# m4rch1n0/vqvae

Measured on AMD Instinct MI355X. Metric: latents/sec through geodesic kNN+APSP+K-medoids, higher is better.
Workload: dtype f64-exact(u32 fixed point)

## Files before the change

vqvae_amd/csrc/geo_common.h:

```cpp
#pragma once
#include <hip/hip_runtime.h>

#include <cstdarg>
#include <cstdint>
#include <cstdio>

#include "geo_hip.h"

namespace geo {

void set_error(const char *fmt, ...);

#define GEO_HIP_CHECK(expr)                                                                      \
    do {                                                                                         \
        hipError_t _e = (expr);                                                                  \
        if (_e != hipSuccess) {                                                                  \
            geo::set_error("%s failed: %s (%s:%d)", #expr, hipGetErrorString(_e), __FILE__, __LINE__); \
            return GEO_E_HIP;                                                                    \
        }                                                                                        \
    } while (0)

#define GEO_REQUIRE(cond, ...)              \
    do {                                    \
        if (!(cond)) {                      \
            geo::set_error(__VA_ARGS__);    \
            return GEO_E_ARG;               \
        }                                   \
    } while (0)

#define GEO_LAUNCH_CHECK() GEO_HIP_CHECK(hipGetLastError())

struct Options {
    int sssp_sb = -1, sssp_act = 1, sssp_sparse_div = -1, sssp_map_div = -1, sssp_group = 1, sssp_grouped_cap = 256,
        sssp_trace = 0, sssp_u32 = 1, sssp_push = 1 ,
        sssp_delta = 8 , sssp_order = 0 , sssp_push_blocks = 64, knn_filter = 1, kpp_grid = 256, kpp_profile = 0, jvp_mid = 0 ,
        jvp_back_valu = 0, jvp_front_valu = 0, jvp_per_node = 1 ,
        jvp_pipe_grid = 1 ,
        jvp_node_jacobian = 1 ,
        jvp_start_dedup = 1 ;
};
Options &options();

static inline size_t align_up(size_t x, size_t a = 256) { return (x + a - 1) / a * a; }

struct Arena {
    char *base;
    size_t size, off;
    Arena(void *p, size_t n) : base(static_cast<char *>(p)), size(n), off(0) {}
    template <typename T>
    T *take(size_t count) {
        size_t bytes = align_up(count * sizeof(T));
        if (off + bytes > size) return nullptr;
        T *r = reinterpret_cast<T *>(base + off);
        off += bytes;
        return r;
    }
};

size_t scan_tmp_bytes(int64_t n);
int exclusive_scan_i32(const int32_t *in, int32_t *out, int64_t n, void *tmp, size_t tmp_bytes,
                       int64_t *total_host, hipStream_t stream);

static inline int grid_for(int64_t work_items, int per_block, int cap = 8192) {
    int64_t g = (work_items + per_block - 1) / per_block;
    if (g < 1) g = 1;
    if (g > cap) g = cap;
    return static_cast<int>(g);
}

}
```

vqvae_amd/csrc/jvp.hip:

```cpp
#include "geo_common.h"

#include <cmath>
#include <cstdlib>
#include <type_traits>
#include <vector>

namespace {

constexpr int TS = 32;
constexpr int NC = 128;
constexpr int MAX_BLOCKS = 4;
constexpr int FRONT_MAX_N1 = 1024;
constexpr int BACK_TS = 8;

typedef float f32x16 __attribute__((ext_vector_type(16)));
typedef __bf16 bf16x8 __attribute__((ext_vector_type(8)));
typedef unsigned short u16x8 __attribute__((ext_vector_type(8)));

struct Shape {
    int d, c0, c1, c2, co, s_out, pad3, p_out;
    int n1, n2;
    int opix_per_chunk, n_chunks;
};

// ... 31 lines not shown
        else b01[n] = (float)(s + (double)b1[co]);
    }
}

__global__ __launch_bounds__(256) void pack_mid_kernel(const float *__restrict__ w2, int c1, int c2, ChunkTable tab,
                                                      int n_chunks, int opix_per_chunk, float *__restrict__ B2p) {
    const size_t per_blk = (size_t)c1 * NC;
    const size_t total = (size_t)n_chunks * MAX_BLOCKS * per_blk;
    for (size_t i = (size_t)blockIdx.x * blockDim.x + threadIdx.x; i < total; i += (size_t)gridDim.x * blockDim.x) {
        const int col = (int)(i % NC);
        const int ci = (int)((i / NC) % c1);
        const int blk = (int)((i / per_blk) % MAX_BLOCKS);
        const int ch = (int)(i / (per_blk * MAX_BLOCKS));
        float v = 0.0f;
        const int lo = col / c2, co = col % c2;
        if (blk < tab.nblk[ch] && lo < opix_per_chunk) {
            const int op = tab.opix[ch][lo], ip = tab.ipix[ch][blk];
            const int ky = (op >> 2) + 1 - 2 * (ip >> 1), kx = (op & 3) + 1 - 2 * (ip & 1);
            if (ky >= 0 && ky < 4 && kx >= 0 && kx < 4) v = w2[(((size_t)ci * c2 + co) * 4 + ky) * 4 + kx];
        }
        B2p[i] = v;
    }
}

__global__ __launch_bounds__(256) void pack_back_kernel(const float *__restrict__ w3, int c2, int co_n,
                                                       float *__restrict__ W3p) {
    const int total = 16 * co_n * c2;
    for (int i = blockIdx.x * blockDim.x + threadIdx.x; i < total; i += gridDim.x * blockDim.x) {
        const int ci = i % c2, co = (i / c2) % co_n, t = i / (c2 * co_n);
        W3p[i] = w3[(((size_t)ci * co_n + co) * 4 + (t >> 2)) * 4 + (t & 3)];
    }
}

template <int DMAX>
__global__ __launch_bounds__(256) void front_kernel(const float *__restrict__ z, const int32_t *__restrict__ src,
                                                   const int32_t *__restrict__ dst, const float *__restrict__ z_start,
                                                   const float *__restrict__ z_end, int64_t e_base, int64_t n_edges,
                                                   int batch, int tiles_per_group, int d, int n1,
                                                   const float *__restrict__ M01, const float *__restrict__ b01,
                                                   float *__restrict__ pre, float *__restrict__ tpre,
                                                   double *__restrict__ partial, int want_stats, int unit_d = 0) {
    __shared__ __attribute__((aligned(8))) float zp[DMAX][TS];
    __shared__ __attribute__((aligned(8))) float dz[DMAX][TS];
    typedef float f32x2 __attribute__((ext_vector_type(2)));
    __shared__ int valid_s[TS];
    __shared__ double ps[FRONT_MAX_N1][4];
    const int tile = blockIdx.x;
    const int group = tile / tiles_per_group, tg = tile % tiles_per_group;
    const int chunk = group >> 1, side = group & 1;
    for (int i = threadIdx.x; i < TS * d; i += 256) {
        const int s = i / d, k = i % d;
        const int within = tg * TS + s;
        const int64_t e = e_base + (int64_t)chunk * batch + within;
        float a = 0.f, b = 0.f;
        const bool ok = within < batch && e < n_edges;
        if (ok) {
            if (src) {
                a = z[(int64_t)src[e] * d + k];
                b = z[(int64_t)dst[e] * d + k];
            } else {
                a = z_start[e * d + k];
                b = z_end[e * d + k];
            }
        }
        zp[k][s] = side == 0 ? a : b;
        dz[k][s] = unit_d ? ((ok && k == (int)(e % unit_d)) ? 1.f : 0.f) : b - a;
        if (k == 0) valid_s[s] = ok ? 1 : 0;
    }
    for (int i = threadIdx.x; i < TS * (DMAX - d); i += 256) {
        const int s = i / (DMAX - d), k = d + i % (DMAX - d);
        zp[k][s] = 0.f;
        dz[k][s] = 0.f;
    }
    __syncthreads();
    const size_t slot0 = (size_t)tile * TS;
    for (int n = threadIdx.x; n < n1; n += 256) {
        float m[DMAX];
#pragma unroll
        for (int k = 0; k < DMAX; ++k) m[k] = k < d ? M01[(size_t)k * n1 + n] : 0.f;
        const float bias = b01[n];
        double sx = 0, sxx = 0, st = 0, sxt = 0;
        for (int s = 0; s < TS; s += 2) {
            f32x2 x2 = {bias, bias}, t2 = {0.f, 0.f};
#pragma unroll
            for (int k = 0; k < DMAX; ++k) {
                const f32x2 mk = {m[k], m[k]};
                x2 = __builtin_elementwise_fma(*reinterpret_cast<const f32x2 *>(&zp[k][s]), mk, x2);
                t2 = __builtin_elementwise_fma(*reinterpret_cast<const f32x2 *>(&dz[k][s]), mk, t2);
            }
#pragma unroll
            for (int u = 0; u < 2; ++u) {
                const float x = u ? x2.y : x2.x, t = u ? t2.y : t2.x;
                pre[(slot0 + s + u) * n1 + n] = x;
                tpre[(slot0 + s + u) * n1 + n] = t;
                if (valid_s[s + u]) {
                    sx += x; sxx += (double)x * x; st += t; sxt += (double)x * t;
                }
            }
        }
        if (want_stats) { ps[n][0] = sx; ps[n][1] = sxx; ps[n][2] = st; ps[n][3] = sxt; }
    }
    if (want_stats) {
        __syncthreads();
        const int c1 = n1 / 4;
        for (int c = threadIdx.x; c < c1; c += 256) {
            double a0 = 0, a1 = 0, a2 = 0, a3 = 0;
#pragma unroll
            for (int px = 0; px < 4; ++px) { a0 += ps[px * c1 + c][0]; a1 += ps[px * c1 + c][1]; a2 += ps[px * c1 + c][2]; a3 += ps[px * c1 + c][3]; }
            double *p = partial + ((size_t)tile * c1 + c) * 4;
            p[0] = a0; p[1] = a1; p[2] = a2; p[3] = a3;
        }
    }
}

template <int DMAX>
__global__ __launch_bounds__(256) void front_mfma_kernel(const float *__restrict__ z, const int32_t *__restrict__ src,
                                                        const int32_t *__restrict__ dst, const float *__restrict__ z_start,
                                                        const float *__restrict__ z_end, int64_t e_base, int64_t n_edges,
                                                        int batch, int tiles_per_group, int d, int n1,
                                                        const float *__restrict__ M01, const float *__restrict__ b01,
                                                        float *__restrict__ pre, float *__restrict__ tpre,
                                                        double *__restrict__ partial, int want_stats) {
    __shared__ float zp[TS][DMAX + 1];
    __shared__ float dz[TS][DMAX + 1];
    __shared__ int valid_s[TS];
    __shared__ double ps[FRONT_MAX_N1][4];
    const int tile = blockIdx.x;
    const int group = tile / tiles_per_group, tg = tile % tiles_per_group;
    const int chunk = group >> 1, side = group & 1;
    for (int i = threadIdx.x; i < TS * DMAX; i += 256) {
        const int s = i / DMAX, k = i % DMAX;
        const int within = tg * TS + s;
        const int64_t e = e_base + (int64_t)chunk * batch + within;
        float a = 0.f, b = 0.f;
        const bool ok = within < batch && e < n_edges;
        if (ok && k < d) {
            if (src) {
                a = z[(int64_t)src[e] * d + k];
                b = z[(int64_t)dst[e] * d + k];
            } else {
                a = z_start[e * d + k];
                b = z_end[e * d + k];
            }
        }
// ... 701 lines not shown
#pragma unroll
            for (int w = 0; w < 4; ++w) { a0 += red[w0 + 2 * w][l][0]; a1 += red[w0 + 2 * w][l][1]; a2 += red[w0 + 2 * w][l][2]; a3 += red[w0 + 2 * w][l][3]; }
            double *p = partial2 + ((size_t)tile * c2 + threadIdx.x) * 4;
            p[0] = a0; p[1] = a1; p[2] = a2; p[3] = a3;
        }
    }
#ifdef GEO_MID_PROF
    { const unsigned long long t_e = __builtin_amdgcn_s_memtime();
      GEO_MP_ADD(6, t_e - mp_prev); GEO_MP_ADD(5, mp_wait); GEO_MP_ADD(7, 1); }
#endif
}

struct Bn2Sums { double sx = 0, sxx = 0, st = 0, sxt = 0; };
__device__ __forceinline__ void bn2_add(Bn2Sums &a, float x, float t, bool live) {
    const double xd = live ? (double)x : 0.0, td = live ? (double)t : 0.0;
    a.sx += xd; a.sxx = fma(xd, xd, a.sxx); a.st += td; a.sxt = fma(xd, td, a.sxt);
}
__device__ __forceinline__ void bn2_store(Bn2Sums a, double *__restrict__ partial2, int tile, int wslot, int co, int lane) {
    a.sx += __shfl_xor(a.sx, 32, 64); a.sxx += __shfl_xor(a.sxx, 32, 64);
    a.st += __shfl_xor(a.st, 32, 64); a.sxt += __shfl_xor(a.sxt, 32, 64);
    if (lane < 32) {
        double *pp = partial2 + (((size_t)tile * 4 + wslot) * 64 + co) * 4;
        pp[0] = a.sx; pp[1] = a.sxx; pp[2] = a.st; pp[3] = a.sxt;
    }
}

template <bool END_ONLY>
__global__ __launch_bounds__(512, 2) void mid_pipe_kernel(const float *__restrict__ pre1, const float *__restrict__ tpre1,
                                                         const NormConst *__restrict__ consts1, int consts_per_group,
                                                         int tiles_per_group, int n_tiles, int ,
                                                         const unsigned short *__restrict__ B3, const float *__restrict__ b2,
                                                         float *__restrict__ pre2, float *__restrict__ tpre2,
                                                         double *__restrict__ partial2, int want_stats, int64_t e_base,
                                                         int64_t n_edges, int batch) {
    constexpr int C1 = 128, LDK = C1 + 8, KS = C1 / 16, NL = 4, c2 = 64;
    typedef float f32x2 __attribute__((ext_vector_type(2)));
    __shared__ __attribute__((aligned(16))) unsigned short A3[2][3][2][TS][LDK];
    const int lane = threadIdx.x & 63, wave = __builtin_amdgcn_readfirstlane((int)(threadIdx.x >> 6));
    const int wq = wave & 3, wg = wave >> 2;
    constexpr int n1 = 4 * C1, n2 = 16 * c2;
    const int r = lane & 31, h = lane >> 5;
    const int k0p = 2 * lane;
    const int lo = wq >> 1, co = (wq & 1) * 32 + r;
    const float bias = b2[co];
    const unsigned v_out = (unsigned)(4 * h * n2 + co) * 4u;
    const int my_tiles = (n_tiles - (int)blockIdx.x + (int)gridDim.x - 1) / (int)gridDim.x;
    if (my_tiles <= 0) return;

    f32x16 accp[NL], acct[NL];
    auto zero_acc = [&]() {
#pragma unroll
        for (int lc = 0; lc < NL; ++lc)
#pragma unroll
            for (int i = 0; i < 16; ++i) { accp[lc][i] = 0.f; acct[lc][i] = 0.f; }
    };
    zero_acc();
    NormConst kA, kB;
    f32x2 rp[4], rt[4];
    auto phys = [&](int t) { return END_ONLY ? ((t / tiles_per_group) * 2 + 1) * tiles_per_group + t % tiles_per_group : t; };
    auto load_consts = [&](int tile) {
        tile = phys(tile);
        const NormConst *kp = consts1 + (size_t)(consts_per_group ? tile / tiles_per_group : 0) * C1 + k0p;
        kA = kp[0];
        kB = kp[1];
    };
    const unsigned v_pair = (unsigned)k0p * 4u;
    auto fetch = [&](int tile, int px, int sample0, auto ns_tag) {
        constexpr int NS = decltype(ns_tag)::value;
        const size_t tbase = (size_t)phys(tile) * TS * n1;
        const __amdgpu_buffer_rsrc_t rp_src = __builtin_amdgcn_make_buffer_rsrc(const_cast<float *>(pre1 + tbase), 0, TS * n1 * 4, 0x00020000);
        const __amdgpu_buffer_rsrc_t rt_src = __builtin_amdgcn_make_buffer_rsrc(const_cast<float *>(tpre1 + tbase), 0, TS * n1 * 4, 0x00020000);
        const int soff = (sample0 * n1 + MidGeom::pix(px) * C1) * 4;
#pragma unroll
        for (int i = 0; i < NS; ++i) {
            rp[i] = __builtin_bit_cast(f32x2, __builtin_amdgcn_raw_buffer_load_b64(rp_src, v_pair, soff + i * n1 * 4, 0));
            rt[i] = __builtin_bit_cast(f32x2, __builtin_amdgcn_raw_buffer_load_b64(rt_src, v_pair, soff + i * n1 * 4, 0));
        }
        __builtin_amdgcn_sched_group_barrier(0x020, 2 * NS, 0);
    };
    auto stage = [&](int buf, int sample0, auto ns_tag) {
        constexpr int NS = decltype(ns_tag)::value;
        unsigned w_idx = (unsigned)((buf * 3 * 2 * TS + sample0) * LDK + k0p);
        asm volatile("" : "+v"(w_idx));
        unsigned short *w = &A3[0][0][0][0][0] + w_idx;
#pragma unroll
        for (int i = 0; i < NS; ++i) {
            float a0, t0, a1, t1;
            norm_relu(kA, rp[i].x, rt[i].x, &a0, &t0);
            norm_relu(kB, rp[i].y, rt[i].y, &a1, &t1);
            unsigned wa[3], wt[3];
            split3_pair(a0, a1, wa[0], wa[1], wa[2]);
            split3_pair(t0, t1, wt[0], wt[1], wt[2]);
#pragma unroll
            for (int part = 0; part < 3; ++part) {
                *reinterpret_cast<unsigned *>(w + (part * 2 + 0) * TS * LDK + i * LDK) = wa[part];
                *reinterpret_cast<unsigned *>(w + (part * 2 + 1) * TS * LDK + i * LDK) = wt[part];
            }
        }
    };
    std::integral_constant<int, 4> HALF;
    const int s_half = 4 * wave, s_full = 8 * wq;

    bf16x8 ring[3][3];
    const unsigned b_lane = (unsigned)(h * 3 * NC * 8 + (wq * 32 + r) * 8) * 2u;
// ... 111 lines not shown
                                                        int slots_per_group, int32_t *__restrict__ row_map, int32_t *__restrict__ rep,
                                                        int32_t *__restrict__ n_compact) {
    __shared__ int wsum[4];
    __shared__ int carry_s;
    const int chunk = blockIdx.x;
    const size_t g0 = (size_t)chunk * 2 * slots_per_group;
    const int lane = threadIdx.x & 63, wave = threadIdx.x >> 6;
    int carry = 0;
    for (int w0 = 0; w0 < slots_per_group; w0 += 256) {
        const int within = w0 + (int)threadIdx.x;
        const int64_t e = e_base + (int64_t)chunk * batch + within;
        const bool valid = within < slots_per_group && within < batch && e < n_edges;
        const bool head = valid && (within == 0 || src[e] != src[e - 1]);
        const unsigned long long m = __ballot(head);
        const int below = __popcll(m & ((1ull << lane) - 1ull));
        if (lane == 0) wsum[wave] = __popcll(m);
        __syncthreads();
        int before = carry, total = carry;
        for (int w = 0; w < 4; ++w) { if (w < wave) before += wsum[w]; total += wsum[w]; }
        const int k = before + below + (head ? 1 : 0) - 1;
        if (within < slots_per_group) {
            row_map[g0 + within] = (int32_t)(g0 + (valid ? k : 0));
            if (head) rep[g0 + k] = (int32_t)(g0 + within);
        }
        carry = total;
        __syncthreads();
    }
    if (threadIdx.x == 0) { carry_s = carry; n_compact[chunk] = carry; }
    __syncthreads();
    const int cnt = carry_s, padded = (cnt + TS - 1) / TS * TS;
    for (int k = cnt + (int)threadIdx.x; k < padded; k += 256) rep[g0 + k] = (int32_t)g0;
}

template <bool TT>
__global__ __launch_bounds__(512, 2) void mid_start_kernel(const float *__restrict__ pre1, const float *__restrict__ tpre1,
                                                          const NormConst *__restrict__ consts1, int tiles_per_group,
                                                          const unsigned short *__restrict__ B3, const float *__restrict__ b2,
                                                          float *__restrict__ pre2, float *__restrict__ tpre2,
                                                          double *__restrict__ partial2, const int32_t *__restrict__ row_map,
                                                          const int32_t *__restrict__ rep, const int32_t *__restrict__ n_compact,
                                                          int64_t e_base, int64_t n_edges, int batch) {
    constexpr int C1 = 128, LDK = C1 + 8, KS = C1 / 16, NL = 4, c2 = 64, n1 = 4 * C1, n2 = 16 * c2;
    typedef float f32x2 __attribute__((ext_vector_type(2)));
    __shared__ __attribute__((aligned(16))) unsigned short A3[2][3][2][TS][LDK];
    const int chunk = blockIdx.y, group = 2 * chunk;
    const int ncomp = TT ? 0 : n_compact[chunk];
    auto run = [&](int item) {
    const int lt0 = 2 * item;
    const bool live1 = TT ? lt0 + 1 < tiles_per_group : (lt0 + 1) * TS < ncomp;
    const int tile0 = group * tiles_per_group + lt0, tile1 = live1 ? tile0 + 1 : tile0;
    const int lane = threadIdx.x & 63, wave = __builtin_amdgcn_readfirstlane((int)(threadIdx.x >> 6));
    const int wq = wave & 3, wg = wave >> 2;
    const int r = lane & 31, h = lane >> 5;
    f32x16 accp[NL], acct[NL];
#pragma unroll
    for (int lc = 0; lc < NL; ++lc)
#pragma unroll
        for (int i = 0; i < 16; ++i) { accp[lc][i] = 0.f; acct[lc][i] = 0.f; }

    const int k0p = 2 * lane, s0p = 4 * wave;
    const NormConst *kp = consts1 + (size_t)group * C1 + k0p;
    const NormConst kA = kp[0], kB = kp[1];
    size_t xrow[2][4];
#pragma unroll
    for (int i = 0; i < 4; ++i) {
        const size_t s0 = (size_t)tile0 * TS + s0p + i, s1 = (size_t)tile1 * TS + s0p + i;
        xrow[0][i] = TT ? s0 : (size_t)__builtin_amdgcn_readfirstlane(rep[s0]);
        xrow[1][i] = TT ? s1 : (size_t)__builtin_amdgcn_readfirstlane(rep[s1]);
    }
    f32x2 rx[2][4], rt[2][4];
    auto fetch = [&](int nx) {
#pragma unroll
        for (int hh = 0; hh < 2; ++hh)
#pragma unroll
            for (int i = 0; i < 4; ++i) {
                const size_t off = xrow[hh][i] * n1 + (size_t)MidGeom::pix(nx) * C1 + k0p;
                rx[hh][i] = *reinterpret_cast<const f32x2 *>(pre1 + off);
                if (TT) rt[hh][i] = *reinterpret_cast<const f32x2 *>(tpre1 + off);
            }
    };
    fetch(0);
    auto stage_px = [&](int buf, int nx) {
#pragma unroll
        for (int hh = 0; hh < 2; ++hh)
#pragma unroll
            for (int i = 0; i < 4; ++i) {
                float a0, t0, a1, t1;
                norm_relu(kA, rx[hh][i].x, TT ? rt[hh][i].x : 0.f, &a0, &t0);
                norm_relu(kB, rx[hh][i].y, TT ? rt[hh][i].y : 0.f, &a1, &t1);
                unsigned w[3];
                if (TT) split3_pair(t0, t1, w[0], w[1], w[2]);
                else split3_pair(a0, a1, w[0], w[1], w[2]);
#pragma unroll
                for (int part = 0; part < 3; ++part) *reinterpret_cast<unsigned *>(&A3[buf][part][hh][s0p + i][k0p]) = w[part];
            }
        if (nx < 4) {
            fetch(nx);
            __builtin_amdgcn_sched_group_barrier(0x020, TT ? 16 : 8, 0);
        }
    };
    bf16x8 ring[3][3];
    const unsigned b_lane = (unsigned)(h * 3 * NC * 8 + (wq * 32 + r) * 8) * 2u;
    const __amdgpu_buffer_rsrc_t b_rsrc = __builtin_amdgcn_make_buffer_rsrc(
        const_cast<unsigned short *>(B3), 0, (int)((size_t)8 * MAX_BLOCKS * C1 * NC * 3 * 2), 0x00020000);
    {
        const int cb0 = wg == 0 ? MidGeom::prod_cb(0, MidGeom::pix(0), 0) : MidGeom::prod_cb(1, MidGeom::pix(0), 0);
        const int cb1 = wg == 0 ? MidGeom::prod_cb(0, MidGeom::pix(0), 1) : MidGeom::prod_cb(1, MidGeom::pix(0), 1);
#pragma unroll
        for (int part = 0; part < 3; ++part) {
            ring[0][part] = __builtin_bit_cast(bf16x8, __builtin_amdgcn_raw_buffer_load_b128(b_rsrc, b_lane, (cb0 * KS * 2 * 3 + part) * NC * 8 * 2, 0));
            ring[1][part] = __builtin_bit_cast(bf16x8, __builtin_amdgcn_raw_buffer_load_b128(b_rsrc, b_lane, (cb1 * KS * 2 * 3 + part) * NC * 8 * 2, 0));
// ... 607 lines not shown
    mid_all_kernel<C1V, GNV><<<(unsigned)nt_node, 512, 0, stream>>>(pre1, tpre1, k1, 0, (int)nt_node, s.c2, B3,         \
                                                                    dc->b2, pre2_node, tpre2, part2, 0, slot_valid,   \
                                                                    gs1, 0, n_nodes, big_batch)
        if (gs1) { if (s.c1 == 128) GEO_MIDA_N(128, true); else if (s.c1 == 64) GEO_MIDA_N(64, true); else GEO_MIDA_N(32, true); }
        else if (s.c1 == 128) GEO_MIDA_N(128, false);
        else if (s.c1 == 64) GEO_MIDA_N(64, false);
        else GEO_MIDA_N(32, false);
#undef GEO_MIDA_N
        GEO_LAUNCH_CHECK();
        if (gs2) {
            group_stats_kernel<<<geo::grid_for((int64_t)node_slots * 32, 256), 256, 0, stream>>>(pre2_node, tpre2, (int64_t)node_slots,
                                                                                                 16, s.c2, 32, dc->eps, gs2);
            GEO_LAUNCH_CHECK();
        }
#define GEO_BACK_N(NTV, GNV)                                                                                       \
    back_mfma_kernel<NTV, GNV, 2><<<(unsigned)nt_node, 256, 0, stream>>>(pre2_node, tpre2, k2, 0, (int)nt_node, s.co,   \
                                                                         s.s_out, W3b, dc->b3, norms, gs2, sg_node)
        if (back_nt == 1) { if (gs2) GEO_BACK_N(1, true); else GEO_BACK_N(1, false); }
        else { if (gs2) GEO_BACK_N(6, true); else GEO_BACK_N(6, false); }
#undef GEO_BACK_N
        GEO_LAUNCH_CHECK();
    }
    const int64_t total_chunks = (n_edges + batch - 1) / batch;
    for (int64_t c0 = 0; c0 < total_chunks; c0 += pl.chunks_per_pass) {
        int64_t nch = total_chunks - c0;
        if (nch > pl.chunks_per_pass) nch = pl.chunks_per_pass;
        const int64_t e_base = c0 * batch;
        int64_t e_count = n_edges - e_base;
        if (e_count > nch * batch) e_count = nch * batch;
        const int64_t p_groups = nch * 2, p_tiles = p_groups * pl.tiles_per_group, p_slots = p_tiles * TS;
        slot_valid_kernel<<<geo::grid_for(p_slots, 256), 256, 0, stream>>>(e_base, n_edges, batch, pl.tiles_per_group,
                                                                          p_slots, slot_valid);
        GEO_LAUNCH_CHECK();
#define GEO_FRONT(DM)                                                                                              \
    front_kernel<DM><<<(unsigned)p_tiles, 256, 0, stream>>>(z, src, dst, z_start, z_end, e_base, n_edges, batch,    \
                                                            pl.tiles_per_group, s.d, s.n1, M01, b01, pre1, tpre1,   \
                                                            part1, batch_stats ? 1 : 0, unit_d)
#define GEO_FRONT_MFMA(DM)                                                                                         \
    front_mfma_kernel<DM><<<(unsigned)p_tiles, 256, 0, stream>>>(z, src, dst, z_start, z_end, e_base, n_edges, batch, \
                                                                 pl.tiles_per_group, s.d, s.n1, M01, b01, pre1,       \
                                                                 tpre1, part1, batch_stats ? 1 : 0)
        const bool front_mfma = s.d > 16 && s.n1 % 32 == 0 && geo::options().jvp_front_valu == 0;
        if (s.d <= 16) { if (geo::options().jvp_front_valu == 2 && s.n1 % 32 == 0 && !unit_d) GEO_FRONT_MFMA(16); else GEO_FRONT(16); }
        else if (s.d <= 32) { if (front_mfma) GEO_FRONT_MFMA(32); else GEO_FRONT(32); }
        else { if (front_mfma) GEO_FRONT_MFMA(64); else GEO_FRONT(64); }
#undef GEO_FRONT_MFMA
#undef GEO_FRONT
        GEO_LAUNCH_CHECK();
        if (batch_stats) {
            finalize_batch_kernel<<<geo::grid_for(p_groups * s.c1, 256), 256, 0, stream>>>(
                part1, pl.tiles_per_group, 1, 4, s.c1, e_base, n_edges, batch, dc->g1, dc->be1, dc->eps, k1, (int)p_groups,
                track ? stats : nullptr);
            if (track)
                running_update_kernel<<<(unsigned)((s.c1 + 7) / 8), 256, 0, stream>>>(stats, (int)p_groups, s.c1, dc->momentum,
                                                                          const_cast<float *>(dc->rm1), const_cast<float *>(dc->rv1));
            GEO_LAUNCH_CHECK();
        }
        if (gs1) {
            group_stats_kernel<<<geo::grid_for(p_slots * 32, 256), 256, 0, stream>>>(pre1, tpre1, p_slots, 4, s.c1, 32,
                                                                                    dc->eps, gs1);
            GEO_LAUNCH_CHECK();
        }
        const dim3 mgrid((unsigned)p_tiles, (unsigned)s.n_chunks);
#define GEO_MID(C1V)                                                                                               \
    mid_kernel<C1V><<<mgrid, 256, 0, stream>>>(pre1, tpre1, k1, batch_stats ? 1 : 0, pl.tiles_per_group, tab,       \
                                               s.opix_per_chunk, s.c2, B2p, dc->b2, pre2, tpre2, part2,             \
                                               batch_stats ? 1 : 0, slot_valid)
#define GEO_MID3(C1V)                                                                                              \
    mid_bf16_kernel<C1V><<<mgrid, 256, 0, stream>>>(pre1, tpre1, k1, batch_stats ? 1 : 0, pl.tiles_per_group, tab,  \
                                                    s.opix_per_chunk, s.c2, B3, dc->b2, pre2, tpre2, part2,        \
                                                    batch_stats ? 1 : 0, slot_valid)
        const bool mid_all = mid_split && s.n_chunks == 8 && s.opix_per_chunk == 2 && s.c1 >= 32 &&
                             mid_opt != 2;
        const bool mid_pipe = mid_all && !per_node && !gs1 && s.c1 == 128 && s.c2 == 64 && mid_opt != 3;
        const size_t np_back = (size_t)back_nt * 32;
        const bool dedup = batch_stats && src && dst && mid_pipe && back_mfma && !jac_node && !gs2 &&
                           geo::options().jvp_start_dedup != 0 && (2 * slots + groups) * 4 <= tiles * s.n1 * 4 * 8 &&
                           np_back <= (size_t)s.n1;
        int32_t *row_map = reinterpret_cast<int32_t *>(part1), *rep = row_map + slots, *n_compact = rep + slots;
        float *sg_compact = pre1;
        const int64_t side_tiles = nch * pl.tiles_per_group;
        if (dedup) {
            start_runs_kernel<<<(unsigned)nch, 256, 0, stream>>>(src, e_base, n_edges, batch, pl.slots_per_group, row_map, rep,
                                                                 n_compact);
            GEO_LAUNCH_CHECK();
        }
        if (mid_all && per_node) {
#define GEO_MIDA_T(C1V, GNV)                                                                                       \
    mid_all_kernel<C1V, GNV, true><<<(unsigned)p_tiles, 512, 0, stream>>>(pre1, tpre1, k1, 0, pl.tiles_per_group,       \
                                                                          s.c2, B3, dc->b2, pre2, tpre2, part2, 0,     \
                                                                          slot_valid, gs1, e_base, n_edges, batch)
            if (gs1) { if (s.c1 == 128) GEO_MIDA_T(128, true); else if (s.c1 == 64) GEO_MIDA_T(64, true); else GEO_MIDA_T(32, true); }
            else if (s.c1 == 128) GEO_MIDA_T(128, false);
            else if (s.c1 == 64) GEO_MIDA_T(64, false);
            else GEO_MIDA_T(32, false);
#undef GEO_MIDA_T
        } else if (mid_pipe) {
            static int n_cu = 0;
            if (n_cu == 0) {
                int devid = 0;
                hipDeviceProp_t prop;
                GEO_HIP_CHECK(hipGetDevice(&devid));
                GEO_HIP_CHECK(hipGetDeviceProperties(&prop, devid));
                n_cu = prop.multiProcessorCount > 0 ? prop.multiProcessorCount : 256;
            }
            const int per_cu = geo::options().jvp_pipe_grid > 0 ? geo::options().jvp_pipe_grid : 1;
            const int64_t pipe_tiles = dedup ? side_tiles : p_tiles;
            const unsigned pgrid = (unsigned)std::min<int64_t>(pipe_tiles, (int64_t)n_cu * per_cu);
#define GEO_PIPE(EO)                                                                                               \
    mid_pipe_kernel<EO><<<pgrid, 512, 0, stream>>>(pre1, tpre1, k1, batch_stats ? 1 : 0, pl.tiles_per_group, (int)pipe_tiles, \
                                                   s.c2, B3, dc->b2, pre2, tpre2, part2, batch_stats ? 1 : 0, e_base,  \
                                                   n_edges, batch)
            if (dedup) GEO_PIPE(true);
            else GEO_PIPE(false);
#undef GEO_PIPE
            if (dedup) {
                const dim3 sgrid((unsigned)((pl.tiles_per_group + 1) / 2), (unsigned)nch);
                mid_start_kernel<false><<<dim3(1, (unsigned)nch), 512, 0, stream>>>(pre1, tpre1, k1, pl.tiles_per_group, B3, dc->b2, pre2, tpre2,
                                                                   part2, row_map, rep, n_compact, e_base, n_edges, batch);
                GEO_LAUNCH_CHECK();
                mid_start_kernel<true><<<sgrid, 512, 0, stream>>>(pre1, tpre1, k1, pl.tiles_per_group, B3, dc->b2, pre2, tpre2,
                                                                  part2, row_map, rep, n_compact, e_base, n_edges, batch);
            }
        } else if (mid_all) {
#define GEO_MIDA(C1V, GNV)                                                                                         \
    mid_all_kernel<C1V, GNV><<<(unsigned)p_tiles, 512, 0, stream>>>(pre1, tpre1, k1, batch_stats ? 1 : 0,           \
                                                                    pl.tiles_per_group, s.c2, B3, dc->b2,           \
                                                                    pre2, tpre2, part2, batch_stats ? 1 : 0,        \
                                                                    slot_valid, gs1, e_base, n_edges, batch)
            if (gs1) {
                if (s.c1 == 128) GEO_MIDA(128, true);
                else if (s.c1 == 64) GEO_MIDA(64, true);
                else GEO_MIDA(32, true);
            } else if (s.c1 == 128) GEO_MIDA(128, false);
            else if (s.c1 == 64) GEO_MIDA(64, false);
            else GEO_MIDA(32, false);
#undef GEO_MIDA
        } else if (mid_split) {
            if (s.c1 == 128) GEO_MID3(128);
            else if (s.c1 == 64) GEO_MID3(64);
            else GEO_MID3(32);
        } else {
            if (s.c1 == 128) GEO_MID(128);
            else if (s.c1 == 64) GEO_MID(64);
            else GEO_MID(32);
        }
#undef GEO_MID3
#undef GEO_MID
        GEO_LAUNCH_CHECK();
        if (batch_stats) {
            finalize_batch_kernel<<<geo::grid_for(p_groups * s.c2, 256), 256, 0, stream>>>(
                part2, pl.tiles_per_group, mid_pipe ? 4 : (mid_all ? 1 : 16), 16, s.c2, e_base, n_edges, batch, dc->g2, dc->be2, dc->eps, k2, (int)p_groups,
                track ? stats : nullptr);
            if (track)
                running_update_kernel<<<(unsigned)((s.c2 + 7) / 8), 256, 0, stream>>>(stats, (int)p_groups, s.c2, dc->momentum,
// ... 148 lines not shown
```

vqvae_amd/csrc/common.hip:

```cpp
#include "geo_common.h"

#include <cstdlib>
#include <cstring>

namespace geo {

namespace {
struct OptionName { const char *name, *env; int Options::*field; };
const OptionName kOptionNames[] = {
    {"sssp_sb", "GEO_SSSP_SB", &Options::sssp_sb},
    {"sssp_act", "GEO_SSSP_ACT", &Options::sssp_act},
    {"sssp_sparse_div", "GEO_SSSP_SPARSE_DIV", &Options::sssp_sparse_div},
    {"sssp_map_div", "GEO_SSSP_MAP_DIV", &Options::sssp_map_div},
    {"sssp_group", "GEO_SSSP_GROUP", &Options::sssp_group},
    {"sssp_grouped_cap", "GEO_SSSP_GROUPED_CAP", &Options::sssp_grouped_cap},
    {"sssp_trace", "GEO_SSSP_TRACE", &Options::sssp_trace},
    {"sssp_u32", "GEO_SSSP_U32", &Options::sssp_u32},
    {"sssp_push", "GEO_SSSP_PUSH", &Options::sssp_push},
    {"sssp_order", "GEO_SSSP_ORDER", &Options::sssp_order},
    {"sssp_delta", "GEO_SSSP_DELTA", &Options::sssp_delta},
    {"sssp_push_blocks", "GEO_SSSP_PUSH_BLOCKS", &Options::sssp_push_blocks},
    {"knn_filter", "GEO_KNN_FILTER", &Options::knn_filter},
    {"kpp_grid", "GEO_KPP_GRID", &Options::kpp_grid},
    {"kpp_profile", "GEO_KPP_PROFILE", &Options::kpp_profile},
    {"jvp_mid", "GEO_JVP_MID", &Options::jvp_mid},
    {"jvp_back_valu", "GEO_JVP_BACK_VALU", &Options::jvp_back_valu},
    {"jvp_front_valu", "GEO_JVP_FRONT_VALU", &Options::jvp_front_valu},
    {"jvp_per_node", "GEO_JVP_PER_NODE", &Options::jvp_per_node},
    {"jvp_node_jacobian", "GEO_JVP_NODE_JACOBIAN", &Options::jvp_node_jacobian},
    {"jvp_pipe_grid", "GEO_JVP_PIPE_GRID", &Options::jvp_pipe_grid},
    {"jvp_start_dedup", "GEO_JVP_START_DEDUP", &Options::jvp_start_dedup},
};
Options from_environment() {
    Options o;
    for (const OptionName &e : kOptionNames) {
        const char *v = getenv(e.env);
        if (!v) continue;
        if (e.field == &Options::jvp_mid) o.jvp_mid = v[0] == 'f' ? 1 : (v[0] == 'c' ? 2 : (v[0] == 'a' ? 3 : atoi(v)));
        else o.*(e.field) = atoi(v);
    }
    return o;
}
}

Options &options() {
    static Options o = from_environment();
    return o;
}

static thread_local char g_err[512] = "";

void set_error(const char *fmt, ...) {
    va_list ap;
    va_start(ap, fmt);
    vsnprintf(g_err, sizeof(g_err), fmt, ap);
    va_end(ap);
}

constexpr int SCAN_THREADS = 256;
constexpr int SCAN_ITEMS = 8;
constexpr int SCAN_TILE = SCAN_THREADS * SCAN_ITEMS;

__global__ __launch_bounds__(SCAN_THREADS) void scan_tiles_kernel(const int32_t *__restrict__ in,
                                                                 int32_t *__restrict__ out,
// ... 114 lines not shown
```

Before: 2.307 million.

## Deduplicate start-point front-layer rows by computing pre-activations once per source run

Adds a front_dedup mode, now on by default, for the side-0 (start) edges in the front kernel. The kernel computes the pre-activation x only at run heads of identical source nodes and writes it to a compacted row, while still writing tangents per slot. mid_start_kernel gains a CP variant that reads pre1 through row_map (or from clamped compact indices) and tpre1 per slot. The dedup run-detection launch and its metadata buffer move ahead of the front kernel, with the buffer offset past the front partials. This removes redundant front-layer arithmetic and pre1 writes for repeated start nodes, at the cost of extra branching and index loads.

Result: no change. 2.325 million (median of 2 runs) (+0.8%).

```diff
diff --git a/vqvae_amd/csrc/geo_common.h b/vqvae_amd/csrc/geo_common.h
--- a/vqvae_amd/csrc/geo_common.h
+++ b/vqvae_amd/csrc/geo_common.h
@@ -37,7 +37,7 @@
         jvp_back_valu = 0, jvp_front_valu = 0, jvp_per_node = 1 ,
         jvp_pipe_grid = 1 ,
         jvp_node_jacobian = 1 ,
-        jvp_start_dedup = 1 ;
+        jvp_start_dedup = 2 ;
 };
 Options &options();
 
diff --git a/vqvae_amd/csrc/jvp.hip b/vqvae_amd/csrc/jvp.hip
--- a/vqvae_amd/csrc/jvp.hip
+++ b/vqvae_amd/csrc/jvp.hip
@@ -87,22 +87,25 @@
     }
 }
 
-template <int DMAX>
+template <int DMAX, bool FD = false>
 __global__ __launch_bounds__(256) void front_kernel(const float *__restrict__ z, const int32_t *__restrict__ src,
                                                    const int32_t *__restrict__ dst, const float *__restrict__ z_start,
                                                    const float *__restrict__ z_end, int64_t e_base, int64_t n_edges,
                                                    int batch, int tiles_per_group, int d, int n1,
                                                    const float *__restrict__ M01, const float *__restrict__ b01,
                                                    float *__restrict__ pre, float *__restrict__ tpre,
-                                                   double *__restrict__ partial, int want_stats, int unit_d = 0) {
+                                                   double *__restrict__ partial, int want_stats, int unit_d = 0,
+                                                   const int32_t *__restrict__ row_map = nullptr) {
     __shared__ __attribute__((aligned(8))) float zp[DMAX][TS];
     __shared__ __attribute__((aligned(8))) float dz[DMAX][TS];
     typedef float f32x2 __attribute__((ext_vector_type(2)));
     __shared__ int valid_s[TS];
+    __shared__ int crow_s[FD ? TS : 1], flag_s[FD ? TS : 1];
     __shared__ double ps[FRONT_MAX_N1][4];
     const int tile = blockIdx.x;
     const int group = tile / tiles_per_group, tg = tile % tiles_per_group;
     const int chunk = group >> 1, side = group & 1;
+    const size_t slot0 = (size_t)tile * TS;
     for (int i = threadIdx.x; i < TS * d; i += 256) {
         const int s = i / d, k = i % d;
         const int within = tg * TS + s;
@@ -121,6 +124,16 @@
         zp[k][s] = side == 0 ? a : b;
         dz[k][s] = unit_d ? ((ok && k == (int)(e % unit_d)) ? 1.f : 0.f) : b - a;
         if (k == 0) valid_s[s] = ok ? 1 : 0;
+        if (FD && k == 0) {
+            int cr = 0, f = 0;
+            if (side == 0 && ok) {
+                cr = row_map[slot0 + s];
+                const bool head = within == 0 || row_map[slot0 + s - 1] != cr;
+                f = head ? 3 : (s == 0 ? 1 : 0);
+            }
+            crow_s[s] = cr;
+            flag_s[s] = f;
+        }
     }
     for (int i = threadIdx.x; i < TS * (DMAX - d); i += 256) {
         const int s = i / (DMAX - d), k = d + i % (DMAX - d);
@@ -128,13 +141,38 @@
         dz[k][s] = 0.f;
     }
     __syncthreads();
-    const size_t slot0 = (size_t)tile * TS;
     for (int n = threadIdx.x; n < n1; n += 256) {
         float m[DMAX];
 #pragma unroll
         for (int k = 0; k < DMAX; ++k) m[k] = k < d ? M01[(size_t)k * n1 + n] : 0.f;
         const float bias = b01[n];
         double sx = 0, sxx = 0, st = 0, sxt = 0;
+        if (FD && side == 0) {
+            float x = 0.f;
+            for (int s = 0; s < TS; s += 2) {
+                f32x2 t2 = {0.f, 0.f};
+#pragma unroll
+                for (int k = 0; k < DMAX; ++k) {
+                    const f32x2 mk = {m[k], m[k]};
+                    t2 = __builtin_elementwise_fma(*reinterpret_cast<const f32x2 *>(&dz[k][s]), mk, t2);
+                }
+#pragma unroll
+                for (int u = 0; u < 2; ++u) {
+                    const int f = flag_s[s + u];
+                    if (f & 1) {
+                        x = bias;
+#pragma unroll
+                        for (int k = 0; k < DMAX; ++k) x = __builtin_fmaf(zp[k][s + u], m[k], x);
+                    }
+                    if (f & 2) pre[(size_t)crow_s[s + u] * n1 + n] = x;
+                    const float t = u ? t2.y : t2.x;
+                    tpre[(slot0 + s + u) * n1 + n] = t;
+                    if (valid_s[s + u]) {
+                        sx += x; sxx += (double)x * x; st += t; sxt += (double)x * t;
+                    }
+                }
+            }
+        } else
         for (int s = 0; s < TS; s += 2) {
             f32x2 x2 = {bias, bias}, t2 = {0.f, 0.f};
 #pragma unroll
@@ -1147,7 +1185,7 @@
     for (int k = cnt + (int)threadIdx.x; k < padded; k += 256) rep[g0 + k] = (int32_t)g0;
 }
 
-template <bool TT>
+template <bool TT, bool CP>
 __global__ __launch_bounds__(512, 2) void mid_start_kernel(const float *__restrict__ pre1, const float *__restrict__ tpre1,
                                                           const NormConst *__restrict__ consts1, int tiles_per_group,
                                                           const unsigned short *__restrict__ B3, const float *__restrict__ b2,
@@ -1176,12 +1214,20 @@
     const int k0p = 2 * lane, s0p = 4 * wave;
     const NormConst *kp = consts1 + (size_t)group * C1 + k0p;
     const NormConst kA = kp[0], kB = kp[1];
-    size_t xrow[2][4];
+    size_t xrow[2][4], trow[2][4];
+    const size_t last_c = (size_t)group * tiles_per_group * TS + (size_t)(ncomp > 0 ? ncomp - 1 : 0);
 #pragma unroll
     for (int i = 0; i < 4; ++i) {
         const size_t s0 = (size_t)tile0 * TS + s0p + i, s1 = (size_t)tile1 * TS + s0p + i;
-        xrow[0][i] = TT ? s0 : (size_t)__builtin_amdgcn_readfirstlane(rep[s0]);
-        xrow[1][i] = TT ? s1 : (size_t)__builtin_amdgcn_readfirstlane(rep[s1]);
+        trow[0][i] = s0;
+        trow[1][i] = s1;
+        if (CP) {
+            xrow[0][i] = TT ? (size_t)__builtin_amdgcn_readfirstlane(row_map[s0]) : (s0 < last_c ? s0 : last_c);
+            xrow[1][i] = TT ? (size_t)__builtin_amdgcn_readfirstlane(row_map[s1]) : (s1 < last_c ? s1 : last_c);
+        } else {
+            xrow[0][i] = TT ? s0 : (size_t)__builtin_amdgcn_readfirstlane(rep[s0]);
+            xrow[1][i] = TT ? s1 : (size_t)__builtin_amdgcn_readfirstlane(rep[s1]);
+        }
     }
     f32x2 rx[2][4], rt[2][4];
     auto fetch = [&](int nx) {
@@ -1189,9 +1235,9 @@
         for (int hh = 0; hh < 2; ++hh)
 #pragma unroll
             for (int i = 0; i < 4; ++i) {
-                const size_t off = xrow[hh][i] * n1 + (size_t)MidGeom::pix(nx) * C1 + k0p;
-                rx[hh][i] = *reinterpret_cast<const f32x2 *>(pre1 + off);
-                if (TT) rt[hh][i] = *reinterpret_cast<const f32x2 *>(tpre1 + off);
+                const size_t col = (size_t)MidGeom::pix(nx) * C1 + k0p;
+                rx[hh][i] = *reinterpret_cast<const f32x2 *>(pre1 + xrow[hh][i] * n1 + col);
+                if (TT) rt[hh][i] = *reinterpret_cast<const f32x2 *>(tpre1 + trow[hh][i] * n1 + col);
             }
     };
     fetch(0);
@@ -1874,7 +1920,28 @@
                                                                  pl.tiles_per_group, s.d, s.n1, M01, b01, pre1,       \
                                                                  tpre1, part1, batch_stats ? 1 : 0)
         const bool front_mfma = s.d > 16 && s.n1 % 32 == 0 && geo::options().jvp_front_valu == 0;
-        if (s.d <= 16) { if (geo::options().jvp_front_valu == 2 && s.n1 % 32 == 0 && !unit_d) GEO_FRONT_MFMA(16); else GEO_FRONT(16); }
+        const bool front_mfma16 = geo::options().jvp_front_valu == 2 && s.n1 % 32 == 0 && !unit_d;
+        const bool mid_all = mid_split && s.n_chunks == 8 && s.opix_per_chunk == 2 && s.c1 >= 32 &&
+                             mid_opt != 2;
+        const bool mid_pipe = mid_all && !per_node && !gs1 && s.c1 == 128 && s.c2 == 64 && mid_opt != 3;
+        const size_t np_back = (size_t)back_nt * 32;
+        const bool dedup = batch_stats && src && dst && mid_pipe && back_mfma && !jac_node && !gs2 &&
+                           geo::options().jvp_start_dedup != 0 && (2 * slots + groups) * 4 <= tiles * (size_t)(s.n1 - s.c1) * 4 * 8 &&
+                           np_back <= (size_t)s.n1;
+        const bool front_dedup = dedup && geo::options().jvp_start_dedup >= 2 && s.d <= 16 && !front_mfma16;
+        int32_t *row_map = reinterpret_cast<int32_t *>(part1 + tiles * s.c1 * 4), *rep = row_map + slots, *n_compact = rep + slots;
+        float *sg_compact = pre1;
+        const int64_t side_tiles = nch * pl.tiles_per_group;
+        if (dedup) {
+            start_runs_kernel<<<(unsigned)nch, 256, 0, stream>>>(src, e_base, n_edges, batch, pl.slots_per_group, row_map, rep,
+                                                                 n_compact);
+            GEO_LAUNCH_CHECK();
+        }
+        if (front_dedup)
+            front_kernel<16, true><<<(unsigned)p_tiles, 256, 0, stream>>>(z, src, dst, z_start, z_end, e_base, n_edges, batch,
+                                                                          pl.tiles_per_group, s.d, s.n1, M01, b01, pre1, tpre1,
+                                                                          part1, 1, 0, row_map);
+        else if (s.d <= 16) { if (front_mfma16) GEO_FRONT_MFMA(16); else GEO_FRONT(16); }
         else if (s.d <= 32) { if (front_mfma) GEO_FRONT_MFMA(32); else GEO_FRONT(32); }
         else { if (front_mfma) GEO_FRONT_MFMA(64); else GEO_FRONT(64); }
 #undef GEO_FRONT_MFMA
@@ -1903,21 +1970,6 @@
     mid_bf16_kernel<C1V><<<mgrid, 256, 0, stream>>>(pre1, tpre1, k1, batch_stats ? 1 : 0, pl.tiles_per_group, tab,  \
                                                     s.opix_per_chunk, s.c2, B3, dc->b2, pre2, tpre2, part2,        \
                                                     batch_stats ? 1 : 0, slot_valid)
-        const bool mid_all = mid_split && s.n_chunks == 8 && s.opix_per_chunk == 2 && s.c1 >= 32 &&
-                             mid_opt != 2;
-        const bool mid_pipe = mid_all && !per_node && !gs1 && s.c1 == 128 && s.c2 == 64 && mid_opt != 3;
-        const size_t np_back = (size_t)back_nt * 32;
-        const bool dedup = batch_stats && src && dst && mid_pipe && back_mfma && !jac_node && !gs2 &&
-                           geo::options().jvp_start_dedup != 0 && (2 * slots + groups) * 4 <= tiles * s.n1 * 4 * 8 &&
-                           np_back <= (size_t)s.n1;
-        int32_t *row_map = reinterpret_cast<int32_t *>(part1), *rep = row_map + slots, *n_compact = rep + slots;
-        float *sg_compact = pre1;
-        const int64_t side_tiles = nch * pl.tiles_per_group;
-        if (dedup) {
-            start_runs_kernel<<<(unsigned)nch, 256, 0, stream>>>(src, e_base, n_edges, batch, pl.slots_per_group, row_map, rep,
-                                                                 n_compact);
-            GEO_LAUNCH_CHECK();
-        }
         if (mid_all && per_node) {
 #define GEO_MIDA_T(C1V, GNV)                                                                                       \
     mid_all_kernel<C1V, GNV, true><<<(unsigned)p_tiles, 512, 0, stream>>>(pre1, tpre1, k1, 0, pl.tiles_per_group,       \
@@ -1949,11 +2001,15 @@
 #undef GEO_PIPE
             if (dedup) {
                 const dim3 sgrid((unsigned)((pl.tiles_per_group + 1) / 2), (unsigned)nch);
-                mid_start_kernel<false><<<dim3(1, (unsigned)nch), 512, 0, stream>>>(pre1, tpre1, k1, pl.tiles_per_group, B3, dc->b2, pre2, tpre2,
-                                                                   part2, row_map, rep, n_compact, e_base, n_edges, batch);
+#define GEO_MID_START(TTV, CPV, GRID)                                                                              \
+    mid_start_kernel<TTV, CPV><<<GRID, 512, 0, stream>>>(pre1, tpre1, k1, pl.tiles_per_group, B3, dc->b2, pre2, tpre2, \
+                                                         part2, row_map, rep, n_compact, e_base, n_edges, batch)
+                if (front_dedup) GEO_MID_START(false, true, dim3(1, (unsigned)nch));
+                else GEO_MID_START(false, false, dim3(1, (unsigned)nch));
                 GEO_LAUNCH_CHECK();
-                mid_start_kernel<true><<<sgrid, 512, 0, stream>>>(pre1, tpre1, k1, pl.tiles_per_group, B3, dc->b2, pre2, tpre2,
-                                                                  part2, row_map, rep, n_compact, e_base, n_edges, batch);
+                if (front_dedup) GEO_MID_START(true, true, sgrid);
+                else GEO_MID_START(true, false, sgrid);
+#undef GEO_MID_START
             }
         } else if (mid_all) {
 #define GEO_MIDA(C1V, GNV)                                                                                         \
```

## Compute both edge endpoints' front layer in one kernel sharing tangent

Applied to the files above, without the earlier changes.

Adds a front_edge_kernel that loads src and dst latents for each edge tile together and computes both sides' first-layer pre-activations in one pass. The tangent (dst - src) projection is computed and stored once, on the src side only. The mid pipe kernel then redirects tangent reads for odd groups to the partner tile's buffer. This removes duplicated tangent computation and writes, and one of the two front-tile launches per edge pair. It adds pointer-offset tricks (tpre1 - t_back) that are only valid under a narrow set of conditions, so a wrong offset would silently read the wrong tile.

Result: no change. 2.304 million before, 2.329 million after, median of 6 (+1.1%).

```diff
diff --git a/vqvae_amd/csrc/common.hip b/vqvae_amd/csrc/common.hip
--- a/vqvae_amd/csrc/common.hip
+++ b/vqvae_amd/csrc/common.hip
@@ -30,6 +30,7 @@
     {"jvp_node_jacobian", "GEO_JVP_NODE_JACOBIAN", &Options::jvp_node_jacobian},
     {"jvp_pipe_grid", "GEO_JVP_PIPE_GRID", &Options::jvp_pipe_grid},
     {"jvp_start_dedup", "GEO_JVP_START_DEDUP", &Options::jvp_start_dedup},
+    {"jvp_front_shared", "GEO_JVP_FRONT_SHARED", &Options::jvp_front_shared},
 };
 Options from_environment() {
     Options o;
diff --git a/vqvae_amd/csrc/geo_common.h b/vqvae_amd/csrc/geo_common.h
--- a/vqvae_amd/csrc/geo_common.h
+++ b/vqvae_amd/csrc/geo_common.h
@@ -37,7 +37,8 @@
         jvp_back_valu = 0, jvp_front_valu = 0, jvp_per_node = 1 ,
         jvp_pipe_grid = 1 ,
         jvp_node_jacobian = 1 ,
-        jvp_start_dedup = 1 ;
+        jvp_start_dedup = 1 ,
+        jvp_front_shared = 1 ;
 };
 Options &options();
 
diff --git a/vqvae_amd/csrc/jvp.hip b/vqvae_amd/csrc/jvp.hip
--- a/vqvae_amd/csrc/jvp.hip
+++ b/vqvae_amd/csrc/jvp.hip
@@ -165,6 +165,87 @@
             double *p = partial + ((size_t)tile * c1 + c) * 4;
             p[0] = a0; p[1] = a1; p[2] = a2; p[3] = a3;
         }
+    }
+}
+
+constexpr int FRONT_EDGE_N1 = 512;
+template <int DMAX>
+__global__ __launch_bounds__(256) void front_edge_kernel(const float *__restrict__ z, const int32_t *__restrict__ src,
+                                                        const int32_t *__restrict__ dst, int64_t e_base, int64_t n_edges,
+                                                        int batch, int tiles_per_group, int d, int n1,
+                                                        const float *__restrict__ M01, const float *__restrict__ b01,
+                                                        float *__restrict__ pre, float *__restrict__ tpre,
+                                                        double *__restrict__ partial) {
+    __shared__ __attribute__((aligned(8))) float za[DMAX][TS];
+    __shared__ __attribute__((aligned(8))) float zb[DMAX][TS];
+    __shared__ __attribute__((aligned(8))) float dz[DMAX][TS];
+    typedef float f32x2 __attribute__((ext_vector_type(2)));
+    __shared__ int valid_s[TS];
+    __shared__ double ps[2][FRONT_EDGE_N1][4];
+    const int chunk = blockIdx.x / tiles_per_group, tg = blockIdx.x % tiles_per_group;
+    const int tile_a = 2 * chunk * tiles_per_group + tg, tile_b = tile_a + tiles_per_group;
+    for (int i = threadIdx.x; i < TS * d; i += 256) {
+        const int s = i / d, k = i % d;
+        const int within = tg * TS + s;
+        const int64_t e = e_base + (int64_t)chunk * batch + within;
+        float a = 0.f, b = 0.f;
+        const bool ok = within < batch && e < n_edges;
+        if (ok) {
+            a = z[(int64_t)src[e] * d + k];
+            b = z[(int64_t)dst[e] * d + k];
+        }
+        za[k][s] = a;
+        zb[k][s] = b;
+        dz[k][s] = b - a;
+        if (k == 0) valid_s[s] = ok ? 1 : 0;
+    }
+    for (int i = threadIdx.x; i < TS * (DMAX - d); i += 256) {
+        const int s = i / (DMAX - d), k = d + i % (DMAX - d);
+        za[k][s] = 0.f;
+        zb[k][s] = 0.f;
+        dz[k][s] = 0.f;
+    }
+    __syncthreads();
+    const size_t slot_a = (size_t)tile_a * TS, slot_b = (size_t)tile_b * TS;
+    for (int n = threadIdx.x; n < n1; n += 256) {
+        float m[DMAX];
+#pragma unroll
+        for (int k = 0; k < DMAX; ++k) m[k] = k < d ? M01[(size_t)k * n1 + n] : 0.f;
+        const float bias = b01[n];
+        double ax = 0, axx = 0, at = 0, axt = 0, bx = 0, bxx = 0, bt = 0, bxt = 0;
+        for (int s = 0; s < TS; s += 2) {
+            f32x2 xa2 = {bias, bias}, xb2 = {bias, bias}, t2 = {0.f, 0.f};
+#pragma unroll
+            for (int k = 0; k < DMAX; ++k) {
+                const f32x2 mk = {m[k], m[k]};
+                xa2 = __builtin_elementwise_fma(*reinterpret_cast<const f32x2 *>(&za[k][s]), mk, xa2);
+                xb2 = __builtin_elementwise_fma(*reinterpret_cast<const f32x2 *>(&zb[k][s]), mk, xb2);
+                t2 = __builtin_elementwise_fma(*reinterpret_cast<const f32x2 *>(&dz[k][s]), mk, t2);
+            }
+#pragma unroll
+            for (int u = 0; u < 2; ++u) {
+                const float xa = u ? xa2.y : xa2.x, xb = u ? xb2.y : xb2.x, t = u ? t2.y : t2.x;
+                pre[(slot_a + s + u) * n1 + n] = xa;
+                pre[(slot_b + s + u) * n1 + n] = xb;
+                tpre[(slot_a + s + u) * n1 + n] = t;
+                if (valid_s[s + u]) {
+                    ax += xa; axx += (double)xa * xa; at += t; axt += (double)xa * t;
+                    bx += xb; bxx += (double)xb * xb; bt += t; bxt += (double)xb * t;
+                }
+            }
+        }
+        ps[0][n][0] = ax; ps[0][n][1] = axx; ps[0][n][2] = at; ps[0][n][3] = axt;
+        ps[1][n][0] = bx; ps[1][n][1] = bxx; ps[1][n][2] = bt; ps[1][n][3] = bxt;
+    }
+    __syncthreads();
+    const int c1 = n1 / 4;
+    for (int i = threadIdx.x; i < 2 * c1; i += 256) {
+        const int side = i / c1, c = i % c1;
+        double a0 = 0, a1 = 0, a2 = 0, a3 = 0;
+#pragma unroll
+        for (int px = 0; px < 4; ++px) { a0 += ps[side][px * c1 + c][0]; a1 += ps[side][px * c1 + c][1]; a2 += ps[side][px * c1 + c][2]; a3 += ps[side][px * c1 + c][3]; }
+        double *p = partial + ((size_t)(side ? tile_b : tile_a) * c1 + c) * 4;
+        p[0] = a0; p[1] = a1; p[2] = a2; p[3] = a3;
     }
 }
 
@@ -932,7 +1013,7 @@
                                                          const unsigned short *__restrict__ B3, const float *__restrict__ b2,
                                                          float *__restrict__ pre2, float *__restrict__ tpre2,
                                                          double *__restrict__ partial2, int want_stats, int64_t e_base,
-                                                         int64_t n_edges, int batch) {
+                                                         int64_t n_edges, int batch, int t_partner) {
     constexpr int C1 = 128, LDK = C1 + 8, KS = C1 / 16, NL = 4, c2 = 64;
     typedef float f32x2 __attribute__((ext_vector_type(2)));
     __shared__ __attribute__((aligned(16))) unsigned short A3[2][3][2][TS][LDK];
@@ -967,9 +1048,11 @@
     const unsigned v_pair = (unsigned)k0p * 4u;
     auto fetch = [&](int tile, int px, int sample0, auto ns_tag) {
         constexpr int NS = decltype(ns_tag)::value;
-        const size_t tbase = (size_t)phys(tile) * TS * n1;
+        const int ptile = phys(tile);
+        const int ttile = !END_ONLY && ((ptile / tiles_per_group) & 1) ? ptile - t_partner : ptile;
+        const size_t tbase = (size_t)ptile * TS * n1, ttbase = (size_t)ttile * TS * n1;
         const __amdgpu_buffer_rsrc_t rp_src = __builtin_amdgcn_make_buffer_rsrc(const_cast<float *>(pre1 + tbase), 0, TS * n1 * 4, 0x00020000);
-        const __amdgpu_buffer_rsrc_t rt_src = __builtin_amdgcn_make_buffer_rsrc(const_cast<float *>(tpre1 + tbase), 0, TS * n1 * 4, 0x00020000);
+        const __amdgpu_buffer_rsrc_t rt_src = __builtin_amdgcn_make_buffer_rsrc(const_cast<float *>(tpre1 + ttbase), 0, TS * n1 * 4, 0x00020000);
         const int soff = (sample0 * n1 + MidGeom::pix(px) * C1) * 4;
 #pragma unroll
         for (int i = 0; i < NS; ++i) {
@@ -1865,6 +1948,9 @@
         slot_valid_kernel<<<geo::grid_for(p_slots, 256), 256, 0, stream>>>(e_base, n_edges, batch, pl.tiles_per_group,
                                                                           p_slots, slot_valid);
         GEO_LAUNCH_CHECK();
+        const bool mid_all = mid_split && s.n_chunks == 8 && s.opix_per_chunk == 2 && s.c1 >= 32 &&
+                             mid_opt != 2;
+        const bool mid_pipe = mid_all && !per_node && !gs1 && s.c1 == 128 && s.c2 == 64 && mid_opt != 3;
 #define GEO_FRONT(DM)                                                                                              \
     front_kernel<DM><<<(unsigned)p_tiles, 256, 0, stream>>>(z, src, dst, z_start, z_end, e_base, n_edges, batch,    \
                                                             pl.tiles_per_group, s.d, s.n1, M01, b01, pre1, tpre1,   \
@@ -1874,7 +1960,13 @@
                                                                  pl.tiles_per_group, s.d, s.n1, M01, b01, pre1,       \
                                                                  tpre1, part1, batch_stats ? 1 : 0)
         const bool front_mfma = s.d > 16 && s.n1 % 32 == 0 && geo::options().jvp_front_valu == 0;
-        if (s.d <= 16) { if (geo::options().jvp_front_valu == 2 && s.n1 % 32 == 0 && !unit_d) GEO_FRONT_MFMA(16); else GEO_FRONT(16); }
+        const bool front_shared = batch_stats && src && dst && mid_pipe && back_mfma && !jac_node && s.d <= 16 &&
+                                  s.n1 == FRONT_EDGE_N1 && geo::options().jvp_front_valu != 2 &&
+                                  geo::options().jvp_front_shared != 0;
+        if (front_shared)
+            front_edge_kernel<16><<<(unsigned)(nch * pl.tiles_per_group), 256, 0, stream>>>(
+                z, src, dst, e_base, n_edges, batch, pl.tiles_per_group, s.d, s.n1, M01, b01, pre1, tpre1, part1);
+        else if (s.d <= 16) { if (geo::options().jvp_front_valu == 2 && s.n1 % 32 == 0 && !unit_d) GEO_FRONT_MFMA(16); else GEO_FRONT(16); }
         else if (s.d <= 32) { if (front_mfma) GEO_FRONT_MFMA(32); else GEO_FRONT(32); }
         else { if (front_mfma) GEO_FRONT_MFMA(64); else GEO_FRONT(64); }
 #undef GEO_FRONT_MFMA
@@ -1903,9 +1995,6 @@
     mid_bf16_kernel<C1V><<<mgrid, 256, 0, stream>>>(pre1, tpre1, k1, batch_stats ? 1 : 0, pl.tiles_per_group, tab,  \
                                                     s.opix_per_chunk, s.c2, B3, dc->b2, pre2, tpre2, part2,        \
                                                     batch_stats ? 1 : 0, slot_valid)
-        const bool mid_all = mid_split && s.n_chunks == 8 && s.opix_per_chunk == 2 && s.c1 >= 32 &&
-                             mid_opt != 2;
-        const bool mid_pipe = mid_all && !per_node && !gs1 && s.c1 == 128 && s.c2 == 64 && mid_opt != 3;
         const size_t np_back = (size_t)back_nt * 32;
         const bool dedup = batch_stats && src && dst && mid_pipe && back_mfma && !jac_node && !gs2 &&
                            geo::options().jvp_start_dedup != 0 && (2 * slots + groups) * 4 <= tiles * s.n1 * 4 * 8 &&
@@ -1940,10 +2029,11 @@
             const int per_cu = geo::options().jvp_pipe_grid > 0 ? geo::options().jvp_pipe_grid : 1;
             const int64_t pipe_tiles = dedup ? side_tiles : p_tiles;
             const unsigned pgrid = (unsigned)std::min<int64_t>(pipe_tiles, (int64_t)n_cu * per_cu);
+            const size_t t_back = front_shared ? (size_t)pl.slots_per_group * s.n1 : 0;
 #define GEO_PIPE(EO)                                                                                               \
-    mid_pipe_kernel<EO><<<pgrid, 512, 0, stream>>>(pre1, tpre1, k1, batch_stats ? 1 : 0, pl.tiles_per_group, (int)pipe_tiles, \
+    mid_pipe_kernel<EO><<<pgrid, 512, 0, stream>>>(pre1, EO ? tpre1 - t_back : tpre1, k1, batch_stats ? 1 : 0, pl.tiles_per_group, (int)pipe_tiles, \
                                                    s.c2, B3, dc->b2, pre2, tpre2, part2, batch_stats ? 1 : 0, e_base,  \
-                                                   n_edges, batch)
+                                                   n_edges, batch, front_shared ? pl.tiles_per_group : 0)
             if (dedup) GEO_PIPE(true);
             else GEO_PIPE(false);
 #undef GEO_PIPE
```
